# xswang/xflow

Measured on AMD Instinct MI355X. Metric: examples/sec, higher is better.
Workload: dtype f32

## Files before the change

include/xflow_amd.h:

```cpp
#ifndef XFLOW_AMD_H_
#define XFLOW_AMD_H_

#include <stddef.h>
#include <stdint.h>

#ifdef __cplusplus
extern "C" {
#endif

#define XF_OK 0
#define XF_EINVAL 1
#define XF_EHIP 2
#define XF_EFULL 3
#define XF_EIO 4
#define XF_EPARSE 5
#define XF_ENOGPU 6

const char *xf_last_error(void);
int xf_version(void);
int xf_device_count(int *count);

uint64_t xf_hash_bytes(const void *ptr, size_t len);
int xf_hash_decimal_range(uint64_t start, size_t n, uint64_t *out);
int xf_hash_decimal_ids(const uint64_t *ids, size_t n, uint64_t *out);
// ... 359 lines not shown
                   const int32_t *fgid, const float *vals, const int32_t *labels,
                   size_t row_begin, size_t row_end, void *stream, const uint64_t **d_keys_out,
                   const int32_t **d_fgid_out, const float **d_vals_out,
                   const uint32_t **d_rowptr_out, const int32_t **d_labels_out, uint32_t *R_out,
                   uint32_t *NNZ_out);
int xf_admit_export(xf_admit *a, uint8_t *counters);
int xf_admit_import(xf_admit *a, const uint8_t *counters);
int xf_admit_save(xf_admit *a, const char *path);
int xf_admit_load(xf_admit *a, const char *path);
int xf_admit_stats(const xf_admit *a, uint64_t *nonzeros_seen, uint64_t *nonzeros_kept);

typedef struct xf_negsample xf_negsample;
int xf_negsample_create(xf_negsample **out, float keep, uint64_t seed);
int xf_negsample_destroy(xf_negsample *s);
int xf_negsample_params(const xf_negsample *s, float *keep, uint64_t *seed);
int xf_negsample_weight(const xf_negsample *s, float *weight);
int xf_negsample_keep(uint64_t seed, uint64_t stream, uint64_t ordinal, float keep);
int xf_negsample_apply_dev(xf_negsample *s, uint64_t stream_id, uint64_t first_ordinal,
                           const uint64_t *d_keys, const int32_t *d_fgid, const float *d_vals,
                           const uint32_t *d_rowptr, const int32_t *d_labels, uint32_t R,
                           uint32_t NNZ, void *stream, const uint64_t **d_keys_out,
                           const int32_t **d_fgid_out, const float **d_vals_out,
                           const uint32_t **d_rowptr_out, const int32_t **d_labels_out,
                           uint32_t *R_out, uint32_t *NNZ_out);
int xf_negsample_apply(xf_negsample *s, uint64_t stream_id, uint64_t first_ordinal,
                       const uint64_t *rowptr, const uint64_t *keys, const int32_t *fgid,
                       const float *vals, const int32_t *labels, size_t row_begin, size_t row_end,
                       void *stream, const uint64_t **d_keys_out, const int32_t **d_fgid_out,
                       const float **d_vals_out, const uint32_t **d_rowptr_out,
                       const int32_t **d_labels_out, uint32_t *R_out, uint32_t *NNZ_out);
int xf_negsample_stats(const xf_negsample *s, uint64_t *rows_seen, uint64_t *rows_kept,
                       uint64_t *neg_seen, uint64_t *neg_kept);
int xf_workspace_neg_weight(xf_workspace *ws, float weight);
int xf_sharded_set_neg_weight(xf_sharded *st, float weight);

int xf_auc_logloss(const int32_t *labels, const float *pctr, size_t n,
                   float *acc_logloss_inout, float *auc, int *tp, int *fp,
                   double *nat_logloss);

int XFCreate(void **h, const char *train_path, const char *test_path);
int XFStartTrain(void **h);
int XFDestroy(void **h);
int XFSetParam(void *h, const char *name, const char *value);
int XFGetMetric(void *h, const char *name, double *value);
int XFSaveModel(void *h, const char *path);
int XFLoadModel(void *h, const char *path);
int XFPredict(void *h);
int XFGetTables(void *h, xf_table **w, xf_table **v);

#ifdef __cplusplus
}
#endif
#endif
```

xflow_amd/capi.py:

```python
import collections
import ctypes as C
import os

import numpy as np

_HERE = os.path.dirname(os.path.abspath(__file__))
LIB_PATH = os.environ.get("XF_LIB") or os.path.join(_HERE, "lib", "libxflow_amd.so")

XF_OK = 0
OPT_FTRL, OPT_SGD = 0, 1
INIT_ZERO, INIT_CONST, INIT_HASHNORM = 0, 1, 2
(DEFRAG_NONE, DEFRAG_SORTFREE, DEFRAG_RADIX_ASKED, DEFRAG_RADIX_EXTENT, DEFRAG_RADIX_COUNT,
 DEFRAG_RADIX_CLUSTER) = range(6)
HEAVY_SEG = 64
FM_REFERENCE, FM_CANONICAL, FM_FIELD_AWARE = 0, 1, 2
FM_MODES = {"reference": FM_REFERENCE, "canonical": FM_CANONICAL, "field_aware": FM_FIELD_AWARE}

u64p = C.POINTER(C.c_uint64)
u32p = C.POINTER(C.c_uint32)
i32p = C.POINTER(C.c_int32)
f32p = C.POINTER(C.c_float)
vp = C.c_void_p


# ... 223 lines not shown
    "xf_admit_range": (C.c_int, [C.c_int, C.c_int, C.c_int, u64p, u64p]),
    "xf_admit_range_of": (C.c_int, [vp, u64p, u64p]),
    "xf_admit_destroy": (C.c_int, [vp]),
    "xf_admit_params": (C.c_int, [vp, C.POINTER(C.c_int), C.POINTER(C.c_int), C.POINTER(C.c_int),
                                  C.POINTER(C.c_uint64)]),
    "xf_admit_apply_dev": (C.c_int, [vp, C.c_int, vp, vp, vp, vp, C.c_uint32, C.c_uint32, vp,
                                     C.POINTER(vp), C.POINTER(vp), C.POINTER(vp), C.POINTER(vp),
                                     C.POINTER(C.c_uint32)]),
    "xf_admit_apply": (C.c_int, [vp, C.c_int, u64p, u64p, i32p, f32p, i32p, C.c_size_t,
                                 C.c_size_t, vp, C.POINTER(vp), C.POINTER(vp), C.POINTER(vp),
                                 C.POINTER(vp), C.POINTER(vp), C.POINTER(C.c_uint32),
                                 C.POINTER(C.c_uint32)]),
    "xf_admit_export": (C.c_int, [vp, C.POINTER(C.c_uint8)]),
    "xf_admit_import": (C.c_int, [vp, C.POINTER(C.c_uint8)]),
    "xf_admit_save": (C.c_int, [vp, C.c_char_p]),
    "xf_admit_load": (C.c_int, [vp, C.c_char_p]),
    "xf_admit_stats": (C.c_int, [vp, u64p, u64p]),
    "xf_negsample_create": (C.c_int, [C.POINTER(vp), C.c_float, C.c_uint64]),
    "xf_negsample_destroy": (C.c_int, [vp]),
    "xf_negsample_params": (C.c_int, [vp, C.POINTER(C.c_float), u64p]),
    "xf_negsample_weight": (C.c_int, [vp, C.POINTER(C.c_float)]),
    "xf_negsample_keep": (C.c_int, [C.c_uint64, C.c_uint64, C.c_uint64, C.c_float]),
    "xf_negsample_apply_dev": (C.c_int, [vp, C.c_uint64, C.c_uint64, vp, vp, vp, vp, vp,
                                         C.c_uint32, C.c_uint32, vp, C.POINTER(vp),
                                         C.POINTER(vp), C.POINTER(vp), C.POINTER(vp),
                                         C.POINTER(vp), C.POINTER(C.c_uint32),
                                         C.POINTER(C.c_uint32)]),
    "xf_negsample_apply": (C.c_int, [vp, C.c_uint64, C.c_uint64, u64p, u64p, i32p, f32p, i32p,
                                     C.c_size_t, C.c_size_t, vp, C.POINTER(vp), C.POINTER(vp),
                                     C.POINTER(vp), C.POINTER(vp), C.POINTER(vp),
                                     C.POINTER(C.c_uint32), C.POINTER(C.c_uint32)]),
    "xf_negsample_stats": (C.c_int, [vp, u64p, u64p, u64p, u64p]),
    "xf_workspace_neg_weight": (C.c_int, [vp, C.c_float]),
    "xf_sharded_set_neg_weight": (C.c_int, [vp, C.c_float]),
    "XFCreate": (C.c_int, [C.POINTER(vp), C.c_char_p, C.c_char_p]),
    "XFStartTrain": (C.c_int, [C.POINTER(vp)]),
    "XFDestroy": (C.c_int, [C.POINTER(vp)]),
    "XFSetParam": (C.c_int, [vp, C.c_char_p, C.c_char_p]),
    "XFGetMetric": (C.c_int, [vp, C.c_char_p, C.POINTER(C.c_double)]),
    "XFGetTables": (C.c_int, [vp, C.POINTER(vp), C.POINTER(vp)]),
    "XFSaveModel": (C.c_int, [vp, C.c_char_p]),
    "XFLoadModel": (C.c_int, [vp, C.c_char_p]),
    "XFPredict": (C.c_int, [vp]),
}

_lib = None


def _share_hip_runtime_with_torch():
    import importlib.util
    import sys
    if "torch" in sys.modules:
        return
    try:
        spec = importlib.util.find_spec("torch")
    except (ImportError, ValueError):
        spec = None
    if spec is None or not spec.origin:
        return
    rt = os.path.join(os.path.dirname(spec.origin), "lib", "libamdhip64.so")
    if os.path.exists(rt):
        try:
            C.CDLL(rt, mode=C.RTLD_GLOBAL)
        except OSError:
            pass

# ... 1108 lines not shown
```

xflow_amd/csrc/xf_batch.cc:

```cpp
#include "xf_batch.h"
#include "xf_scratch.h"
#include "xf_tiling.h"

#include <atomic>
#include <string.h>

#include <algorithm>
#include <cmath>
#include <mutex>
#include <thread>
#include <vector>

namespace {

struct KeyPos {
  uint64_t key;
  uint32_t pos;
};

inline bool keypos_less(const KeyPos &a, const KeyPos &b) {
  return a.key < b.key || (a.key == b.key && a.pos < b.pos);
}

void sort_keypos(std::vector<KeyPos> &a) {
// ... 150 lines not shown
  if (!p) return;
  int dev = 0;
  void *evict = nullptr;
  if (hipGetDevice(&dev) == hipSuccess) {
    std::lock_guard<std::mutex> lk(g_pool_mu);
    if (g_pool_limit > 0) {
      if ((int)g_pool.size() >= g_pool_limit) {
        evict = g_pool.front().p;
        g_pool.erase(g_pool.begin());
      }
      g_pool.push_back({p, bytes, dev, false});
      p = nullptr;
    }
  }
  if (evict) (void)hipFree(evict);
  if (p) (void)hipFree(p);
}

void blob_pool_limit(int blobs) {
  std::vector<Blob> drop;
  {
    std::lock_guard<std::mutex> lk(g_pool_mu);
    g_pool_limit = blobs < 0 ? 0 : blobs;
    while ((int)g_pool.size() > g_pool_limit) {
      drop.push_back(g_pool.back());
      g_pool.pop_back();
    }
  }
  for (const Blob &b : drop) (void)hipFree(b.p);
}
}

namespace xf {
static int g_path[kPathCount] = {0, 0, 0, 0, 0};
int path_switch(int which) { return g_path[which]; }
void set_path_switch(int which, int v) { g_path[which] = v; }
#ifdef XF_EXPERIMENTS
static int g_exp_knob = 0;
int exp_knob() { return g_exp_knob; }
void set_exp_knob(int v) { g_exp_knob = v; }
#endif
static std::atomic<bool> g_device_poisoned{false};
bool device_poisoned() { return g_device_poisoned.load(std::memory_order_relaxed); }
void scratch_poison() { g_device_poisoned.store(true); }
}

extern "C" int xf_batch_pool_reserve(size_t bytes) {
  XF_REQUIRE(bytes > 0, "xf_batch_pool_reserve: no bytes");
  int dev = 0;
  XF_HIP(hipGetDevice(&dev));
  {
    std::lock_guard<std::mutex> lk(xf::g_pool_mu);
    if (xf::g_pool_limit <= 0) return XF_OK;
    for (const xf::Blob &b : xf::g_pool)
      if (b.reserved && b.dev == dev && b.bytes >= bytes) return XF_OK;
  }
  void *p = nullptr;
  XF_HIP(hipMalloc(&p, bytes));
  std::lock_guard<std::mutex> lk(xf::g_pool_mu);
  xf::g_pool.push_back({p, bytes, dev, true});
  return XF_OK;
}

extern "C" int xf_scratch_reserve(size_t bytes) {
  xf::Arena &a = xf::arena();
  XF_REQUIRE(a.used == 0, "xf_scratch_reserve: a build is in progress on this thread");
  if (bytes <= a.cap) return XF_OK;
  if (a.base) XF_HIP(hipFree(a.base));
  a.base = nullptr;
  a.cap = 0;
  XF_HIP(hipMalloc((void **)&a.base, bytes));
  a.cap = bytes;
  return XF_OK;
}

extern "C" int xf_tune(const char *name, double value) {
  XF_REQUIRE(name, "xf_tune: null name");
  if (!strcmp(name, "panel_slice_bytes")) g_panel_slice_bytes = value;
  else if (!strcmp(name, "min_panel_nnz")) g_min_panel_nnz = value;
  else if (!strcmp(name, "parse_threads")) xf::set_parse_threads((int)value);
  else if (!strcmp(name, "key_build") && value >= 0 && value <= 3)
    xf::set_path_switch(xf::kPathKeyBuild, (int)value);
  else if (!strcmp(name, "old_weight") && value >= 0 && value <= 2)
    xf::set_path_switch(xf::kPathOldWeight, (int)value);
  else if (!strcmp(name, "lr_gradient") && value >= 0 && value <= 3)
    xf::set_path_switch(xf::kPathLrGradient, (int)value);
  else if (!strcmp(name, "owner_pass") && value >= 0 && value <= 4)
    xf::set_path_switch(xf::kPathOwnerPass, (int)value);
  else if (!strcmp(name, "valued_lr") && (value == 0 || value == 1 || value == 2))
    xf::set_path_switch(xf::kPathValuedLr, (int)value);
#ifdef XF_EXPERIMENTS
  else if (!strcmp(name, "exp_knob")) xf::set_exp_knob((int)value);
#endif
  else if (!strcmp(name, "batch_pool_blobs")) xf::blob_pool_limit((int)value);
  else
    return xf::set_error(XF_EINVAL, "xf_tune: unknown knob '%s' (or a value it does not take)", name);
  return XF_OK;
}

extern "C" int xf_batch_heavy_chunks(const xf_batch *b, uint32_t *H, const uint32_t **chunk_ptr) {
  XF_REQUIRE(b && H, "xf_batch_heavy_chunks: null argument");
  XF_TRY(need_host(b));
  *H = b->H;
  if (chunk_ptr) *chunk_ptr = b->hchunk_ptr.data();
  return XF_OK;
}

extern "C" int xf_batch_tiles(const xf_batch *b, uint32_t *ntiles, const uint32_t **tile_ptr) {
  XF_REQUIRE(b && ntiles, "xf_batch_tiles: null argument");
  XF_TRY(need_host(b));
  *ntiles = (uint32_t)(b->tile_ptr.size() - 1);
  if (tile_ptr) *tile_ptr = b->tile_ptr.data();
  return XF_OK;
}

extern "C" int xf_batch_fwd_tiles(const xf_batch *b, uint32_t *ntiles, const uint32_t **tile_ptr,
                                  const uint32_t **panel_first, uint32_t *grid) {
  XF_REQUIRE(b && ntiles, "xf_batch_fwd_tiles: null argument");
  XF_TRY(need_host(b));
// ... 307 lines not shown
```

xflow_amd/csrc/xf_cells.h:

```cpp
#ifndef XF_CELLS_H_
#define XF_CELLS_H_

#include <stdint.h>

#include "xf_common.h"

namespace xf {

#ifndef XF_CHUNK_BITS
#define XF_CHUNK_BITS 11
#endif
#ifndef XF_WIN_MAX
#define XF_WIN_MAX 17408
#endif
constexpr int kChunkBits = XF_CHUNK_BITS;
constexpr uint32_t kChunk = 1u << kChunkBits;
constexpr uint32_t kWinMax = XF_WIN_MAX;
constexpr uint32_t kRowMask = 0x7FFFu;
constexpr int kTagShift = kChunkBits + 15 > 27 ? kChunkBits + 15 : 27;
constexpr uint32_t kTagMask = (1u << (32 - kTagShift)) - 1u;
static_assert(kChunkBits >= 8 && kChunkBits <= 13, "chunk of 256 .. 8192 index positions");
constexpr uint32_t kBlk = 1024;
#ifndef XF_SLICE_MAX
#define XF_SLICE_MAX (4 * kChunk > 8192 ? 4 * kChunk : 8192)
// ... 31 lines not shown
  uint8_t *item_done = nullptr;
  double *gsum = nullptr;
  uint8_t *gtouched = nullptr;
  size_t split_bytes = 0;
  mutable bool split_dirty = true;
};

namespace xf {

int cells_build(xf_cells **out, const uint32_t *d_src, const uint32_t *d_map,
                const uint32_t *d_rowptr, uint32_t R, uint32_t NNZ, uint32_t M, int mode,
                bool key_sorted_copy, hipStream_t stream, const uint32_t *d_rowid = nullptr,
                uint32_t w_fixed = 0, uint32_t chunk0 = 0, const float *d_xval = nullptr);
void cells_free(xf_cells *c);

struct KbDeferred;
int cells_build_keyed(xf_cells **out, xf_table *t, const uint64_t *d_keys,
                      const uint32_t *d_rowptr, const uint32_t *d_rowid, uint32_t R,
                      uint32_t NNZ, bool key_sorted_copy, uint32_t w_fixed, hipStream_t stream,
                      KbDeferred **defer = nullptr);
int cells_build_keyed_finish(KbDeferred *d, hipStream_t stream, bool *more);

int cells_alloc(xf_cells **out, uint32_t R, uint32_t NNZ, uint32_t M, int mode,
                bool key_sorted_copy, uint32_t w_fixed, uint32_t chunk0, bool valued = false);
int cells_plan_items(xf_cells *c, hipStream_t stream);
int cells_fill_items(xf_cells *c, uint32_t nitems, uint32_t nsplit, hipStream_t stream);
int cells_key_sorted_copy(xf_cells *c, hipStream_t stream);
uint32_t cells_split_chunks(const xf_cells *c);

size_t cells_partial_doubles(const xf_cells *c);

int cells_lr_forward(const xf_cells *c, const float *d_w, const int32_t *d_labels,
                     double *d_partial, float *d_loss, float *d_pctr, hipStream_t stream,
                     const xf_cells *resume_from = nullptr);

int cells_sort_valued(const uint32_t *cid, uint32_t *cid_s, const uint32_t *ent,
                      const float *xval, uint32_t n, int bits, uint32_t *entries, float *vals,
                      hipStream_t stream);
int cells_lr_forward_valued(const xf_cells *c, const float *d_w, const int32_t *d_labels,
                            double *d_partial, float *d_loss, float *d_pctr, hipStream_t stream);
int cells_lr_grad_update_valued(const xf_cells *c, const xf_table *t, const float *d_loss,
                                hipStream_t stream);

int cells_lr_forward_sums(const xf_cells *c, const float *d_w, double *d_partial,
                          const uint32_t *d_out_base, const uint32_t *d_out_rows,
                          double *d_rowsum, hipStream_t stream);
int cells_lr_grad_update_sources(const xf_cells *c, const xf_table *t, const float *d_loss,
                                 uint32_t n, const uint32_t *d_win, const uint32_t *d_rows,
                                 const uint32_t *d_loss_base, double *d_gsum,
                                 uint8_t *d_gtouched, hipStream_t stream,
                                 uint32_t rows_if_one = 0 );

}

#endif
```

xflow_amd/csrc/xf_cells_fwd.h:

```cpp
#ifndef XF_CELLS_FWD_H_
#define XF_CELLS_FWD_H_

#include "xf_cells_impl.h"

namespace {
__device__ __forceinline__ uint32_t cell_of(const uint32_t *__restrict__ cellptr, uint32_t lo,
                                            uint32_t hi, uint32_t j) {
  while (lo < hi) {
    const uint32_t mid = lo + (hi - lo + 1) / 2;
    if (cellptr[mid] <= j) lo = mid;
    else
      hi = mid - 1;
  }
  return lo;
}

constexpr int kFwdE = (int)(kBlk / 64);

struct FwdBlock {
  uint32_t ent[kFwdE];
  uint32_t lo, hi;
};

__device__ __forceinline__ void fwd_load(FwdBlock &B, const uint32_t *__restrict__ entries,
                                         const uint32_t *__restrict__ blk_cell, uint32_t b,
                                         uint32_t pb, uint32_t pe, uint32_t lane) {
  B.lo = blk_cell[b];
  B.hi = blk_cell[b + 1];
#pragma unroll
  for (int q = 0; q < kFwdE; ++q) {
    const uint32_t j = b * kBlk + q * 64 + lane;
    B.ent[q] = (j >= pb && j < pe) ? entries[j] : 0xFFFFFFFFu;
  }
}

}

namespace xf {
int cells_lr_finalize(const xf_cells *c, const double *d_partial, const int32_t *d_labels,
                      float *d_loss, float *d_pctr, hipStream_t s);
}

#endif
```

xflow_amd/csrc/xf_cells_fwd.hip:

```cpp
#include "xf_cells_fwd.h"

namespace {
__device__ __forceinline__ void fwd_process(const FwdBlock &B, uint32_t b, uint32_t c0,
                                            uint32_t nchunk, uint32_t lane,
                                            const uint32_t *__restrict__ cellptr,
                                            const float *__restrict__ w, double *wx) {
  const uint32_t lo = B.lo < c0 ? c0 : B.lo;
  const uint32_t hi = B.hi >= c0 + nchunk ? c0 + nchunk - 1 : B.hi;
  const bool near = hi - lo <= kTagMask;
  float wv[kFwdE];
#pragma unroll
  for (int q = 0; q < kFwdE; ++q) {
    const uint32_t e = B.ent[q];
    if (e == 0xFFFFFFFFu) continue;
    const uint32_t cell = near ? lo + (((e >> kTagShift) - (lo - c0)) & kTagMask)
                               : cell_of(cellptr, lo, hi, b * kBlk + q * 64 + lane);
    wv[q] = w[(size_t)(cell - c0) * kChunk + (e & (kChunk - 1))];
  }
#pragma unroll
  for (int q = 0; q < kFwdE; ++q) {
    const uint32_t e = B.ent[q];
    if (e != 0xFFFFFFFFu) atomicAdd(&wx[(e >> kChunkBits) & kRowMask], (double)wv[q]);
  }
}
// ... 10 lines not shown
  double *out = partial + ((size_t)v * G + g) * W;
  for (uint32_t r = tid; r < W; r += kFwdBlock) wx[r] = accumulate ? out[r] : 0.0;
  const uint32_t c0 = v * nchunk;
  const uint32_t wb = cellptr[c0], we = cellptr[c0 + nchunk];
  const uint64_t n = we - wb;
  uint32_t pb = g == 0 ? wb : (uint32_t)((wb + n * g / G) & ~(uint64_t)(kBlk - 1));
  uint32_t pe = g == G - 1 ? we : (uint32_t)((wb + n * (g + 1) / G) & ~(uint64_t)(kBlk - 1));
  if (pb < wb) pb = wb;
  if (pe < pb) pe = pb;
  const uint32_t b_first = pb / kBlk, b_end = pb < pe ? (pe - 1) / kBlk + 1 : b_first;
  if (tid == 0) next_blk = b_first;
  __syncthreads();
  auto grab = [&]() -> uint32_t {
    uint32_t b = 0;
    if (lane == 0) b = atomicAdd(&next_blk, 1u);
    return (uint32_t)__shfl((int)b, 0);
  };
  FwdBlock A, B;
  uint32_t ba = grab(), bb = 0;
  if (ba < b_end) fwd_load(A, entries, blk_cell, ba, pb, pe, lane);
  while (ba < b_end) {
    bb = grab();
    if (bb < b_end) fwd_load(B, entries, blk_cell, bb, pb, pe, lane);
    fwd_process(A, ba, c0, nchunk, lane, cellptr, w, wx);
    if (bb >= b_end) break;
    ba = grab();
    if (ba < b_end) fwd_load(A, entries, blk_cell, ba, pb, pe, lane);
    fwd_process(B, bb, c0, nchunk, lane, cellptr, w, wx);
  }
  __syncthreads();
  for (uint32_t r = tid; r < W; r += kFwdBlock) out[r] = wx[r];
}

__global__ void __launch_bounds__(kBlock)
k_lr_finalize_cells(const double *__restrict__ partial, const int32_t *__restrict__ labels,
                    uint32_t R, uint32_t W, uint32_t G, float *__restrict__ loss,
                    float *__restrict__ pctr) {
  const uint32_t t = blockIdx.x * blockDim.x + threadIdx.x;
  const uint32_t r = t >> 2, q = t & 3u;
  double a = 0.0;
  if (r < R) {
    const uint32_t v = r / W, rin = r - v * W;
    const double *p = partial + (size_t)v * G * W + rin;
    double a1 = 0.0, a2 = 0.0, a3 = 0.0;
    uint32_t g = q;
    for (; g + 12 < G; g += 16) {
      a += p[(size_t)g * W];
      a1 += p[(size_t)(g + 4) * W];
      a2 += p[(size_t)(g + 8) * W];
      a3 += p[(size_t)(g + 12) * W];
    }
    for (; g < G; g += 4) a += p[(size_t)g * W];
    a += a1 + (a2 + a3);
  }
  a += __shfl_xor(a, 1);
  a += __shfl_xor(a, 2);
  if (r >= R || q != 0) return;
  const float pr = xf::sigmoid_ref((float)a);
  if (pctr) pctr[r] = pr;
  if (loss) loss[r] = pr - (float)labels[r];
}
}

namespace xf {

int cells_lr_forward(const xf_cells *c, const float *d_w, const int32_t *d_labels,
                     double *d_partial, float *d_loss, float *d_pctr, hipStream_t s,
                     const xf_cells *resume_from) {
  XF_REQUIRE(c && d_w && d_partial && (d_loss || d_pctr), "cells_lr_forward: null argument");
  if (c->R == 0) return XF_OK;
  int acc = 0;
  const xf_cells *first = c;
  if (resume_from) {
    first = resume_from;
    acc = 1;
  }
  for (const xf_cells *q = first; q; q = q->next, acc = 1)
    hipLaunchKernelGGL(k_lr_fwd_cells, dim3(q->nwin * q->G), dim3(kFwdBlock), 0, s, q->fwd_entries(),
                       q->cellptr, q->blk_cell, q->nchunk, q->W, q->G,
                       d_w + (size_t)q->chunk0 * kChunk, d_partial, acc);
  hipLaunchKernelGGL(k_lr_finalize_cells,
                     dim3((unsigned)(((size_t)c->R * 4 + kBlock - 1) / kBlock)), dim3(kBlock), 0, s,
                     d_partial, d_labels, c->R, c->W, c->G, d_loss, d_pctr);
  XF_HIP(hipGetLastError());
  return XF_OK;
}

int cells_lr_finalize(const xf_cells *c, const double *d_partial, const int32_t *d_labels,
                      float *d_loss, float *d_pctr, hipStream_t s) {
  hipLaunchKernelGGL(k_lr_finalize_cells,
                     dim3((unsigned)(((size_t)c->R * 4 + kBlock - 1) / kBlock)), dim3(kBlock), 0, s,
                     d_partial, d_labels, c->R, c->W, c->G, d_loss, d_pctr);
  XF_HIP(hipGetLastError());
  return XF_OK;
}

namespace {
__global__ void __launch_bounds__(kBlock)
k_sum_partials(const double *__restrict__ partial, uint32_t n, uint32_t W, uint32_t G,
               const uint32_t *__restrict__ out_base, const uint32_t *__restrict__ out_rows,
               double *__restrict__ rowsum) {
  const uint32_t t = blockIdx.x * blockDim.x + threadIdx.x;
  const uint32_t r = t >> 2, q = t & 3u;
  const uint32_t v = r < n ? r / W : 0u, rin = r - v * W;
  const bool live = r < n && rin < out_rows[v];
  double a = 0.0;
  if (live) {
    const double *p = partial + (size_t)v * G * W + rin;
    for (uint32_t g = q; g < G; g += 4) a += p[(size_t)g * W];
  }
  a += __shfl_xor(a, 1);
  a += __shfl_xor(a, 2);
  if (live && q == 0) rowsum[out_base[v] + rin] = a;
}
}

int cells_lr_forward_sums(const xf_cells *c, const float *d_w, double *d_partial,
                          const uint32_t *d_out_base, const uint32_t *d_out_rows,
                          double *d_rowsum, hipStream_t s) {
  XF_REQUIRE(c && d_w && d_partial && d_rowsum && d_out_base && d_out_rows,
             "cells_lr_forward_sums: null argument");
  if (c->R == 0) return XF_OK;
  int acc = 0;
  for (const xf_cells *q = c; q; q = q->next, acc = 1)
    hipLaunchKernelGGL(k_lr_fwd_cells, dim3(q->nwin * q->G), dim3(kFwdBlock), 0, s, q->fwd_entries(),
                       q->cellptr, q->blk_cell, q->nchunk, q->W, q->G,
                       d_w + (size_t)q->chunk0 * kChunk, d_partial, acc);
  const uint32_t n = c->nwin * c->W;
  hipLaunchKernelGGL(k_sum_partials, dim3((unsigned)(((size_t)n * 4 + kBlock - 1) / kBlock)),
                     dim3(kBlock), 0, s, d_partial, n, c->W, c->G, d_out_base, d_out_rows,
                     d_rowsum);
  XF_HIP(hipGetLastError());
  return XF_OK;
}

}
```

xflow_amd/csrc/xf_cells_valued.hip:

```cpp
#include <rocprim/device/device_radix_sort.hpp>

#include "xf_cells_fwd.h"
#include "xf_cells_grad.h"

namespace {
__global__ void __launch_bounds__(kBlock)
k_cell_pack_val(const uint32_t *__restrict__ ent, const float *__restrict__ xval, size_t n,
                uint64_t *__restrict__ pay) {
  XF_GRID_STRIDE(j, n)
  pay[j] = ((uint64_t)__float_as_uint(xval[j]) << 32) | ent[j];
}

__global__ void __launch_bounds__(kBlock)
k_cell_split_val(const uint64_t *__restrict__ pay, size_t n, uint32_t *__restrict__ entries,
                 float *__restrict__ vals) {
  XF_GRID_STRIDE(j, n) {
    const uint64_t p = pay[j];
    entries[j] = (uint32_t)p;
    vals[j] = __uint_as_float((uint32_t)(p >> 32));
  }
}

struct FwdBlockV {
  FwdBlock E;
// ... 243 lines not shown
#pragma unroll
    for (int i = 0; i < 8; ++i) {
      if (!t[i]) continue;
      T.w[row0 + kb + i * kBlock + tid] = sw[i];
      if (OPT == XF_OPT_FTRL) xf::store_nz(T, row0 + kb + i * kBlock + tid, sn[i], sz[i]);
    }
  }
}
}

namespace xf {

int cells_sort_valued(const uint32_t *cid, uint32_t *cid_s, const uint32_t *ent,
                      const float *xval, uint32_t n, int bits, uint32_t *entries, float *vals,
                      hipStream_t s) {
  Scratch sc;
  uint64_t *pay = nullptr, *pay_s = nullptr;
  XF_TRY(sc.get(&pay, n));
  XF_TRY(sc.get(&pay_s, n));
  hipLaunchKernelGGL(k_cell_pack_val, dim3(grid_for((size_t)n)), dim3(kBlock), 0, s, ent, xval,
                     (size_t)n, pay);
  size_t tb = 0;
  XF_HIP(rocprim::radix_sort_pairs(nullptr, tb, cid, cid_s, pay, pay_s, (size_t)n, 0, bits, s));
  void *tmp = nullptr;
  XF_TRY(sc.get((char **)&tmp, tb));
  XF_HIP(rocprim::radix_sort_pairs(tmp, tb, cid, cid_s, pay, pay_s, (size_t)n, 0, bits, s));
  hipLaunchKernelGGL(k_cell_split_val, dim3(grid_for((size_t)n)), dim3(kBlock), 0, s, pay_s,
                     (size_t)n, entries, vals);
  XF_HIP(hipGetLastError());
  return XF_OK;
}

int cells_lr_forward_valued(const xf_cells *c, const float *d_w, const int32_t *d_labels,
                            double *d_partial, float *d_loss, float *d_pctr, hipStream_t s) {
  XF_REQUIRE(c && d_w && d_partial && (d_loss || d_pctr),
             "cells_lr_forward_valued: null argument");
  XF_REQUIRE(!c->next && c->chunk0 == 0 && c->entries_k == c->entries && (c->vals || c->NNZ == 0),
             "cells_lr_forward_valued: valued cells are one segment with their values and no "
             "key-sorted copy");
  if (c->R == 0) return XF_OK;
  hipLaunchKernelGGL(k_lr_fwd_cells_valued, dim3(c->nwin * c->G), dim3(kFwdBlock), 0, s, c->entries,
                     c->vals, c->cellptr, c->blk_cell, c->nchunk, c->W, c->G, d_w, d_partial);
  XF_HIP(hipGetLastError());
  return cells_lr_finalize(c, d_partial, d_labels, d_loss, d_pctr, s);
}

int cells_lr_grad_update_valued(const xf_cells *c, const xf_table *t, const float *d_loss,
                                hipStream_t s) {
  XF_REQUIRE(c && t && d_loss, "cells_lr_grad_update_valued: null argument");
  XF_REQUIRE(c->mode == kCellsTableRows, "cells_lr_grad_update_valued: cells are not table rows");
  XF_REQUIRE(!c->next && c->chunk0 == 0 && (c->vals || c->NNZ == 0),
             "cells_lr_grad_update_valued: valued cells are one segment with their values");
  TableDev T = table_dev(t);
  XF_REQUIRE(T.dim == 1, "cells_lr_grad_update_valued: dim must be 1");
  table_note_write(const_cast<xf_table *>(t));
  if (c->nitems == 0) return XF_OK;
  if (path_switch(kPathOldWeight) == 1) T.w_of_nz = false;
  if (c->nsplit_chunks) {
    if (c->split_dirty) XF_HIP(hipMemsetAsync(c->gsum, 0, c->split_bytes, s));
    c->split_dirty = true;
  }
  const int opt = T.nz != nullptr ? XF_OPT_FTRL : XF_OPT_SGD;
  if (opt == XF_OPT_FTRL)
    hipLaunchKernelGGL(k_lr_grad_cells_valued<XF_OPT_FTRL>, dim3(c->nitems), dim3(kBlock), 0, s, T,
                       c->entries, c->vals, c->cellptr, c->nchunk, c->nwin, c->W, c->item_chunk,
                       c->item_slice, c->item_dump, d_loss, c->R, c->M, c->gsum, c->gtouched,
                       c->chunk0);
  else
    hipLaunchKernelGGL(k_lr_grad_cells_valued<XF_OPT_SGD>, dim3(c->nitems), dim3(kBlock), 0, s, T,
                       c->entries, c->vals, c->cellptr, c->nchunk, c->nwin, c->W, c->item_chunk,
                       c->item_slice, c->item_dump, d_loss, c->R, c->M, c->gsum, c->gtouched,
                       c->chunk0);
  XF_HIP(hipGetLastError());
  XF_TRY(cells_launch_split_finish(opt, c, T, s));
  c->split_dirty = false;
  return XF_OK;
}
// ... 3 lines not shown
```

xflow_amd/csrc/xf_common.h:

```cpp
#ifndef XF_COMMON_H_
#define XF_COMMON_H_

#include <hip/hip_runtime_api.h>
#include <stdarg.h>
#include <stdint.h>
#include <stdio.h>

#include "xflow_amd.h"

namespace xf {

int set_error(int code, const char *fmt, ...);
int parse_threads();
void set_parse_threads(int n);
bool device_poisoned();
void scratch_poison();
enum PathSwitch { kPathKeyBuild = 0, kPathOldWeight, kPathLrGradient, kPathOwnerPass,
                  kPathValuedLr, kPathCount };
int path_switch(int which);
void set_path_switch(int which, int v);
inline int key_build_mode() { return path_switch(kPathKeyBuild); }
#ifdef XF_EXPERIMENTS
int exp_knob();
void set_exp_knob(int v);
#endif

#define XF_HIP(expr)                                                                  \
  do {                                                                                \
    hipError_t e__ = (expr);                                                          \
    if (e__ != hipSuccess)                                                            \
      return xf::set_error(XF_EHIP, "%s:%d %s -> %s", __FILE__, __LINE__, #expr,      \
                           hipGetErrorString(e__));                                   \
  } while (0)

#define XF_REQUIRE(cond, ...)                                   \
  do {                                                          \
    if (!(cond)) return xf::set_error(XF_EINVAL, __VA_ARGS__);  \
  } while (0)

#define XF_TRY(expr)           \
  do {                         \
    int rc__ = (expr);         \
    if (rc__ != XF_OK) return rc__; \
  } while (0)

struct ShardRange {
  uint64_t lo;
  uint64_t span;
  uint32_t shard, nshards;
};

// ... 12 lines not shown
```

xflow_amd/csrc/xf_model.hip:

```cpp
#include <hip/hip_runtime.h>

#include <math.h>

#include <algorithm>

#include "xf_batch.h"
#include "xf_cells.h"
#include "xf_common.h"
#include "xf_device.h"
#include "xf_ffm.h"
#include "xf_fm_canonical.h"
#include "xf_negsample.h"
#include "xf_scratch.h"
#include "xf_wave.h"

namespace xf {
const TableDev &table_dev(const xf_table *t);
int table_dim(const xf_table *t);
uint64_t table_uid(const xf_table *t);
uint64_t table_epoch(const xf_table *t);
int table_records(xf_table *t, size_t row_bytes, uint64_t tag, void **rec, uint64_t *gen);
uint64_t table_writes(const xf_table *t);
void table_note_write(xf_table *t);
void table_records_all_set(xf_table *t, const uint64_t key[5]);
// ... 1338 lines not shown
extern "C" int xf_fm_grad_update_dev(xf_table *tw, xf_table *tv, const xf_dev_batch *b,
                                     const uint32_t *d_rows_w, const uint32_t *d_rows_v,
                                     const float *d_wu, const float *d_vu, const float *d_vsum,
                                     const float *d_loss, float *d_gw, float *d_gv, void *stream) {
  return fm_grad_update(tw, tv, b, d_rows_w, d_rows_v, const_cast<float *>(d_wu),
                        const_cast<float *>(d_vu), d_vsum, d_loss, d_gw, d_gv, true, stream);
}

enum { kEvResolve = 0, kEvGather, kEvForward, kEvGrad, kEvUpdate, kEvCount };

struct xf_workspace {
  uint32_t *slots = nullptr, *slots2 = nullptr;
  float *wu = nullptr, *g = nullptr, *vu = nullptr, *gv = nullptr;
  float *loss = nullptr, *pctr = nullptr, *vsum = nullptr;
  void *ks = nullptr;
  void *owner_rec = nullptr;
  size_t capU = 0, capUK = 0, capR = 0;
  double *partial = nullptr;
  size_t capPartial = 0;
  float *gdense = nullptr;
  size_t capGdense = 0;
  bool capture = false;
  int parity = 0;
  int fm_mode = XF_FM_REFERENCE;
  int fm_fields = 0;
  float *fmc_S = nullptr;
  size_t capS = 0;
  float *fmc_vu = nullptr;
  size_t capVu = 0;
  double *fmc_hpart = nullptr;
  size_t capHpart = 0;
  uint32_t lastU = 0, lastR = 0;
  float neg_weight = 1.0f;
  bool profiling = false;
  static constexpr int kEvSets = 8;
  struct EvSet {
    hipEvent_t ev[kEvCount + 1] = {};
    bool pending = false;
    int nseg = 0;
    int seg_slot[kEvCount] = {};
  } sets[kEvSets];
  int cur = 0;
  static constexpr long kProfileEvery = 4;
  long step_no = 0;
  bool rec = false;
  double ms_sum[kEvCount] = {};
  long steps_timed = 0;
  int nmark = 0;
};

static int ws_reserve(xf_workspace *ws, size_t U, size_t UK, size_t R, bool fm_pooled = true) {
  auto grow = [](void **p, size_t bytes) -> hipError_t {
    if (*p) {
      hipError_t e = hipFree(*p);
      if (e != hipSuccess) return e;
    }
    return hipMalloc(p, bytes);
  };
  if (!ws->slots || U > ws->capU) {
    const size_t m = std::max<size_t>(U + U / 8, 1024);
    XF_HIP(grow((void **)&ws->slots, m * 4));
    XF_HIP(grow((void **)&ws->slots2, m * 4));
    XF_HIP(grow((void **)&ws->wu, m * 4));
    XF_HIP(grow((void **)&ws->g, m * 4));
    ws->capU = m;
  }
// ... 196 lines not shown
             "xf_workspace_capture: field-aware FM (xf_workspace_fm_mode) is not stepped with "
             "capture on: its step leaves the pulled weights and the w gradients for "
             "xf_workspace_fetch as it is");
  ws->capture = enable != 0;
  return XF_OK;
}

static int lr_step(xf_table *w, xf_batch *b, xf_workspace *ws, void *stream,
                   xf::KbDeferred *deferred) {
  struct Settle {
    xf::KbDeferred *d;
    void *stream;
    ~Settle() {
      if (d) (void)xf::cells_build_keyed_finish(d, S(stream), nullptr);
    }
  } settle{deferred, stream};
  XF_TRY(xf::ensure_cells(b, w, S(stream)));
  const xf_cells *c = b->cells;
  const bool cap = ws->capture && !b->local && b->d_rows_u;
  if (settle.d && (cap || ws->parity == XF_PARITY_REFERENCE_ORDER)) {
    xf::KbDeferred *d = settle.d;
    settle.d = nullptr;
    XF_TRY(xf::cells_build_keyed_finish(d, S(stream), nullptr));
  }
  XF_TRY(ws_reserve(ws, b->U, 0, b->R));
  XF_TRY(ws_reserve_cells(ws, c, cap));
  ws->rec = ws->profiling && ws->step_no++ % xf_workspace::kProfileEvery == 0;
  if (ws->rec) XF_TRY(ws_next_set(ws));
  ws->lastU = cap ? b->U : 0;
  ws->lastR = b->R;
  const xf::TableDev &T = xf::table_dev(w);
  const int32_t *labels = b->local ? b->raw_labels : b->view.labels;
  XF_BEGIN();
  if (ws->parity == XF_PARITY_REFERENCE_ORDER)
    XF_TRY(lr_forward_reforder(w, b, ws->loss, nullptr, S(stream)));
  else
    XF_TRY(xf::cells_lr_forward(c, T.w, labels, ws->partial, ws->loss, nullptr, S(stream)));
  if (settle.d) {
    xf::KbDeferred *d = settle.d;
    settle.d = nullptr;
    bool more = false;
    XF_TRY(xf::cells_build_keyed_finish(d, S(stream), &more));
    if (more) {
      const size_t had = ws->capPartial;
      XF_TRY(ws_reserve_cells(ws, c, cap));
      XF_TRY(xf::cells_lr_forward(c, xf::table_dev(w).w, labels, ws->partial, ws->loss, nullptr,
                                  S(stream), ws->capPartial == had ? c->next : nullptr));
    }
  }
  XF_TRY(xf::weigh_negatives(ws->loss, labels, b->R, ws->neg_weight, S(stream)));
  XF_END(kEvForward);
  if (cap) XF_TRY(xf::gather_f32(T.w, b->d_rows_u, b->U, ws->wu, S(stream)));
  if (ws->parity == XF_PARITY_REFERENCE_ORDER) {
    XF_TRY(xf::batch_reference_coo(b, S(stream)));
    if (b->U) {
      hipLaunchKernelGGL(k_lr_grad_reforder, dim3(blocks_for_groups(b->U, kBlock / 64)),
                         dim3(kBlock), 0, S(stream), b->view.segptr, b->d_ref_coo, ws->loss, b->U,
                         b->R, ws->g);
      XF_HIP(hipGetLastError());
      XF_TRY(xf_table_update_dev(w, b->d_rows_u, b->U, ws->g, stream));
    }
    XF_END(kEvGrad);
    if (ws->rec) ws->sets[ws->cur].pending = true;
    return XF_OK;
  }
  XF_TRY(xf::cells_lr_grad_update(c, w, ws->loss, cap ? ws->gdense : nullptr, S(stream)));
  XF_END(kEvGrad);
  if (cap) XF_TRY(xf::gather_f32(ws->gdense, b->d_rows_u, b->U, ws->g, S(stream)));
  if (ws->rec) ws->sets[ws->cur].pending = true;
  return XF_OK;
}

static int lr_valued_step(xf_table *w, xf_batch *b, xf_workspace *ws, void *stream);
static int lr_valued_predict(xf_table *w, xf_batch *b, xf_workspace *ws, float *pctr_out);
static int lr_local_valued_step(xf_table *w, xf_batch *b, xf_workspace *ws, void *stream);
static int lr_local_valued_predict(xf_table *w, xf_batch *b, xf_workspace *ws, float *pctr_out);

extern "C" int xf_lr_step(xf_table *w, xf_batch *b, xf_workspace *ws, void *stream) {
  XF_REQUIRE(w && b && ws, "xf_lr_step: null argument");
  XF_REQUIRE(xf::table_dim(w) == 1, "xf_lr_step: the w table must have dim 1");
  if (b->valued) return lr_valued_step(w, b, ws, stream);
  if (b->local_valued) return lr_local_valued_step(w, b, ws, stream);
  return lr_step(w, b, ws, stream, nullptr);
// ... 405 lines not shown
  if (v.U && v.R) {
    xf::table_note_write(w);
    XF_TRY(xf::val_lr_grad_update(w, &v, b->d_coo_val, b->d_fm_rows[0], ws->wu, ws->loss, ws->g,
                                  ws->fmc_hpart, S(stream)));
  }
  XF_END(kEvGrad);
  if (ws->rec) ws->sets[ws->cur].pending = true;
  return XF_OK;
}

static int lr_valued_predict(xf_table *w, xf_batch *b, xf_workspace *ws, float *pctr_out) {
  XF_TRY(valued_check(ws, "xf_lr_predict"));
  XF_TRY(xf_batch_upload(b, nullptr));
  XF_TRY(ws_reserve(ws, b->U, 0, b->R, false));
  const xf_dev_batch &v = b->view;
  XF_TRY(xf_table_pull_dev(w, v.ukeys, v.U, ws->slots, ws->wu, nullptr));
  XF_TRY(xf::val_lr_forward(&v, b->d_xval, ws->wu, ws->loss, ws->pctr, nullptr));
  if (b->R) XF_HIP(hipMemcpy(pctr_out, ws->pctr, (size_t)b->R * 4, hipMemcpyDeviceToHost));
  return xf_table_check(w, nullptr);
}

static int lr_local_valued_step(xf_table *w, xf_batch *b, xf_workspace *ws, void *stream) {
  XF_TRY(valued_check(ws, "xf_lr_step"));
  XF_TRY(xf::ensure_cells(b, w, S(stream)));
  const xf_cells *c = b->cells;
  XF_TRY(ws_reserve(ws, 0, 0, b->R));
  XF_TRY(ws_reserve_cells(ws, c, false));
  ws->rec = ws->profiling && ws->step_no++ % xf_workspace::kProfileEvery == 0;
  if (ws->rec) XF_TRY(ws_next_set(ws));
  ws->lastU = 0;
  ws->lastR = b->R;
  XF_BEGIN();
  XF_TRY(xf::cells_lr_forward_valued(c, xf::table_dev(w).w, b->raw_labels, ws->partial, ws->loss,
                                     nullptr, S(stream)));
  XF_TRY(xf::weigh_negatives(ws->loss, b->raw_labels, b->R, ws->neg_weight, S(stream)));
  XF_END(kEvForward);
  XF_TRY(xf::cells_lr_grad_update_valued(c, w, ws->loss, S(stream)));
  XF_END(kEvGrad);
  if (ws->rec) ws->sets[ws->cur].pending = true;
  return XF_OK;
}

static int lr_local_valued_predict(xf_table *w, xf_batch *b, xf_workspace *ws, float *pctr_out) {
  XF_TRY(valued_check(ws, "xf_lr_predict"));
  XF_TRY(xf::ensure_cells(b, w, nullptr));
  XF_TRY(ws_reserve(ws, 0, 0, b->R));
  XF_TRY(ws_reserve_cells(ws, b->cells, false));
  XF_TRY(xf::cells_lr_forward_valued(b->cells, xf::table_dev(w).w, b->raw_labels, ws->partial,
                                     ws->loss, ws->pctr, nullptr));
  if (b->R) XF_HIP(hipMemcpy(pctr_out, ws->pctr, (size_t)b->R * 4, hipMemcpyDeviceToHost));
  return xf_table_check(w, nullptr);
}

static int no_local_valued(const xf_batch *b, const char *who) {
  XF_REQUIRE(!b->local_valued,
             "%s: a local minibatch with feature values (xf_batch_compile_local_valued*) is "
             "stepped and scored by xf_lr_step / xf_lr_predict only: FM needs a minibatch with a "
             "key list and its value arrays (xf_batch_compile_valued*)", who);
  return XF_OK;
}

extern "C" int xf_fm_step(xf_table *w, xf_table *vt, xf_batch *b, xf_workspace *ws,
                          void *stream) {
  XF_REQUIRE(w && vt && b && ws, "xf_fm_step: null argument");
  XF_REQUIRE(xf::table_dim(w) == 1, "xf_fm_step: the w table must have dim 1");
  XF_TRY(no_local_valued(b, "xf_fm_step"));
  XF_REQUIRE(!b->local, "xf_fm_step: needs a minibatch with a key list (xf_batch_compile*)");
  if (ws->fm_mode == XF_FM_FIELD_AWARE) return fm_field_aware_step(w, vt, b, ws, stream);
// ... 321 lines not shown
```

xflow_amd/csrc/xf_negsample.hip:

```cpp
#include <hip/hip_runtime.h>

#include <rocprim/device/device_scan.hpp>

#include <math.h>

#include <vector>

#include "xf_common.h"
#include "xf_negsample.h"
#include "xflow_amd.h"

namespace {

constexpr int kNsThreads = 256;
constexpr uint32_t kNsTile = 256;
static_assert(kNsTile == kNsThreads, "a row per thread");
constexpr uint32_t kNsChunk = 2048;
constexpr int kNsPerThread = kNsChunk / kNsThreads;

__device__ inline bool ns_row(const uint32_t *__restrict__ rowptr,
                              const int32_t *__restrict__ labels, uint32_t r, uint32_t NNZ,
                              uint64_t base, uint64_t first_ordinal, uint64_t T, bool *negative,
                              uint32_t *len) {
  const uint32_t a = rowptr[r], b = rowptr[r + 1];
  *len = (b >= a && b <= NNZ) ? b - a : 0u;
  *negative = labels[r] == 0;
  return !*negative || xf::negsample_keep_row(base, first_ordinal + (uint64_t)r, T);
}

__device__ inline void ns_block_sum2(uint32_t *a, uint32_t *b, uint32_t (*lds)[kNsThreads / 64]) {
#pragma unroll
  for (int off = 32; off > 0; off >>= 1) {
    *a += __shfl_xor(*a, off, 64);
    *b += __shfl_xor(*b, off, 64);
  }
  const uint32_t t = threadIdx.x;
  if ((t & 63) == 0) {
    lds[0][t >> 6] = *a;
// ... 118 lines not shown
    }
  }
}

__global__ __launch_bounds__(256) void k_weigh_negatives(float *__restrict__ loss,
                                                          const int32_t *__restrict__ labels,
                                                          uint32_t R, float w) {
#pragma clang fp contract(off)
  const uint32_t r = blockIdx.x * blockDim.x + threadIdx.x;
  if (r >= R) return;
  if (labels[r] == 0) loss[r] = w * loss[r];
}

template <typename T>
int grow(T **p, size_t *cap, size_t need) {
  if (need <= *cap && *p) return XF_OK;
  if (*p) XF_HIP(hipFree(*p));
  *p = nullptr;
  *cap = 0;
  const size_t n = need + need / 4 + 64;
  XF_HIP(hipMalloc((void **)p, n * sizeof(T)));
  *cap = n;
  return XF_OK;
}

int check_keep(const char *who, float keep) {
  XF_REQUIRE(isfinite(keep) && keep > 0.0f && keep <= 1.0f,
             "%s: neg_keep must be in (0, 1], not %g", who, (double)keep);
  return XF_OK;
}

}

int xf::weigh_negatives(float *loss, const int32_t *labels, uint32_t R, float w, hipStream_t s) {
  if (w == 1.0f || R == 0) return XF_OK;
  XF_REQUIRE(loss && labels, "weigh_negatives: null argument");
  hipLaunchKernelGGL(k_weigh_negatives, dim3((R + 255) / 256), dim3(256), 0, s, loss, labels, R, w);
  XF_HIP(hipGetLastError());
  return XF_OK;
}

struct xf_negsample {
  float keep = 1.0f;
  uint64_t seed = 0, T = 0;
  uint64_t rows_seen = 0, rows_kept = 0, neg_seen = 0, neg_kept = 0;
  uint64_t *o_keys = nullptr;
  int32_t *o_fgid = nullptr, *o_labels = nullptr;
  float *o_vals = nullptr;
  uint32_t *o_rowptr = nullptr;
  size_t cap_keys = 0, cap_fgid = 0, cap_labels = 0, cap_vals = 0, cap_rowptr = 0;
  uint32_t *src_off = nullptr;
  uint64_t *tile_cnt = nullptr, *tile_off = nullptr;
  size_t cap_src = 0, cap_tcnt = 0, cap_toff = 0;
  char *scan_tmp = nullptr;
  size_t cap_scan = 0;
  unsigned long long *d_stat = nullptr;
  uint64_t *h_back = nullptr;
  uint64_t *u_keys = nullptr;
  int32_t *u_fgid = nullptr, *u_labels = nullptr;
  float *u_vals = nullptr;
  uint32_t *u_rowptr = nullptr;
  size_t ucap_keys = 0, ucap_fgid = 0, ucap_labels = 0, ucap_vals = 0, ucap_rowptr = 0;
  std::vector<uint32_t> h_rowptr;
};

extern "C" int xf_negsample_destroy(xf_negsample *s) {
  if (!s) return XF_OK;
  if (s->d_stat && !xf::device_poisoned()) {
    (void)hipDeviceSynchronize();
    for (void *p : {(void *)s->o_keys, (void *)s->o_fgid, (void *)s->o_labels, (void *)s->o_vals,
                    (void *)s->o_rowptr, (void *)s->src_off, (void *)s->tile_cnt,
                    (void *)s->tile_off, (void *)s->scan_tmp, (void *)s->d_stat, (void *)s->u_keys,
// ... 190 lines not shown
```

Baseline: 470.8 million.

## Fuse negative weighting into LR finalize and prefetch gradient entries in extra blocks

The LR finalize kernel now applies the negative-example loss weight itself, so the separate weigh_negatives launch is no longer needed on the cells path. When a gradient pass follows on a newly seen cell set, the same launch gets extra blocks. These blocks stream the entries_k array with vectorized loads to warm the cache for the gradient kernel. A bit test that can never fire, backed by a static_assert, keeps the compiler from dropping those loads. This costs extra memory traffic and blocks in finalize. A launch counter and a standalone finalize entry point are also exported.

```diff
diff --git a/include/xflow_amd.h b/include/xflow_amd.h
--- a/include/xflow_amd.h
+++ b/include/xflow_amd.h
@@ -415,6 +415,10 @@
 int xf_negsample_stats(const xf_negsample *s, uint64_t *rows_seen, uint64_t *rows_kept,
                        uint64_t *neg_seen, uint64_t *neg_kept);
 int xf_workspace_neg_weight(xf_workspace *ws, float weight);
+uint64_t xf_weigh_negatives_launches(void);
+int xf_cells_finalize_rows(const double *d_partial, const int32_t *d_labels, uint32_t R, uint32_t W,
+                           uint32_t G, float neg_weight, float *d_loss, float *d_pctr,
+                           void *stream);
 int xf_sharded_set_neg_weight(xf_sharded *st, float weight);
 
 int xf_auc_logloss(const int32_t *labels, const float *pctr, size_t n,
diff --git a/xflow_amd/capi.py b/xflow_amd/capi.py
--- a/xflow_amd/capi.py
+++ b/xflow_amd/capi.py
@@ -279,6 +279,9 @@
                                      C.POINTER(C.c_uint32), C.POINTER(C.c_uint32)]),
     "xf_negsample_stats": (C.c_int, [vp, u64p, u64p, u64p, u64p]),
     "xf_workspace_neg_weight": (C.c_int, [vp, C.c_float]),
+    "xf_weigh_negatives_launches": (C.c_uint64, []),
+    "xf_cells_finalize_rows": (C.c_int, [vp, vp, C.c_uint32, C.c_uint32, C.c_uint32, C.c_float,
+                                         vp, vp, vp]),
     "xf_sharded_set_neg_weight": (C.c_int, [vp, C.c_float]),
     "XFCreate": (C.c_int, [C.POINTER(vp), C.c_char_p, C.c_char_p]),
     "XFStartTrain": (C.c_int, [C.POINTER(vp)]),
diff --git a/xflow_amd/csrc/xf_batch.cc b/xflow_amd/csrc/xf_batch.cc
--- a/xflow_amd/csrc/xf_batch.cc
+++ b/xflow_amd/csrc/xf_batch.cc
@@ -206,7 +206,7 @@
 }
 
 namespace xf {
-static int g_path[kPathCount] = {0, 0, 0, 0, 0};
+static int g_path[kPathCount] = {0, 0, 0, 0, 0, 0};
 int path_switch(int which) { return g_path[which]; }
 void set_path_switch(int which, int v) { g_path[which] = v; }
 #ifdef XF_EXPERIMENTS
@@ -259,6 +259,8 @@
     xf::set_path_switch(xf::kPathOldWeight, (int)value);
   else if (!strcmp(name, "lr_gradient") && value >= 0 && value <= 3)
     xf::set_path_switch(xf::kPathLrGradient, (int)value);
+  else if (!strcmp(name, "entry_streams") && (value == 0 || value == 1))
+    xf::set_path_switch(xf::kPathEntryStreams, (int)value);
   else if (!strcmp(name, "owner_pass") && value >= 0 && value <= 4)
     xf::set_path_switch(xf::kPathOwnerPass, (int)value);
   else if (!strcmp(name, "valued_lr") && (value == 0 || value == 1 || value == 2))
diff --git a/xflow_amd/csrc/xf_cells.h b/xflow_amd/csrc/xf_cells.h
--- a/xflow_amd/csrc/xf_cells.h
+++ b/xflow_amd/csrc/xf_cells.h
@@ -87,13 +87,15 @@
 
 int cells_lr_forward(const xf_cells *c, const float *d_w, const int32_t *d_labels,
                      double *d_partial, float *d_loss, float *d_pctr, hipStream_t stream,
-                     const xf_cells *resume_from = nullptr);
+                     const xf_cells *resume_from = nullptr, bool grad_follows = false,
+                     float neg_weight = 1.0f);
 
 int cells_sort_valued(const uint32_t *cid, uint32_t *cid_s, const uint32_t *ent,
                       const float *xval, uint32_t n, int bits, uint32_t *entries, float *vals,
                       hipStream_t stream);
 int cells_lr_forward_valued(const xf_cells *c, const float *d_w, const int32_t *d_labels,
-                            double *d_partial, float *d_loss, float *d_pctr, hipStream_t stream);
+                            double *d_partial, float *d_loss, float *d_pctr, hipStream_t stream,
+                            float neg_weight = 1.0f );
 int cells_lr_grad_update_valued(const xf_cells *c, const xf_table *t, const float *d_loss,
                                 hipStream_t stream);
 
diff --git a/xflow_amd/csrc/xf_cells_fwd.h b/xflow_amd/csrc/xf_cells_fwd.h
--- a/xflow_amd/csrc/xf_cells_fwd.h
+++ b/xflow_amd/csrc/xf_cells_fwd.h
@@ -38,7 +38,7 @@
 
 namespace xf {
 int cells_lr_finalize(const xf_cells *c, const double *d_partial, const int32_t *d_labels,
-                      float *d_loss, float *d_pctr, hipStream_t s);
+                      float *d_loss, float *d_pctr, hipStream_t s, float neg_weight = 1.0f);
 }
 
 #endif
diff --git a/xflow_amd/csrc/xf_cells_fwd.hip b/xflow_amd/csrc/xf_cells_fwd.hip
--- a/xflow_amd/csrc/xf_cells_fwd.hip
+++ b/xflow_amd/csrc/xf_cells_fwd.hip
@@ -66,10 +66,29 @@
   for (uint32_t r = tid; r < W; r += kFwdBlock) out[r] = wx[r];
 }
 
+constexpr uint32_t kFetchVec = 4 * kBlock;
+static_assert(kWinMax <= 0x6000u, "the fetch blocks' impossible entry");
+
 __global__ void __launch_bounds__(kBlock)
 k_lr_finalize_cells(const double *__restrict__ partial, const int32_t *__restrict__ labels,
                     uint32_t R, uint32_t W, uint32_t G, float *__restrict__ loss,
-                    float *__restrict__ pctr) {
+                    float *__restrict__ pctr, float neg_w, uint32_t nfin,
+                    const uint4 *__restrict__ fetch, uint32_t nvec) {
+  if (blockIdx.x >= nfin) {
+    const uint32_t j0 = (blockIdx.x - nfin) * kFetchVec + threadIdx.x;
+    uint4 u[kFetchVec / kBlock];
+#pragma unroll
+    for (int i = 0; i < (int)(kFetchVec / kBlock); ++i) u[i] = fetch[min(j0 + i * kBlock, nvec - 1)];
+    uint32_t bad = 0;
+#pragma unroll
+    for (int i = 0; i < (int)(kFetchVec / kBlock); ++i)
+      bad |= (u[i].x >> 24 & u[i].x >> 25 & ~(u[i].x >> 11)) |
+             (u[i].y >> 24 & u[i].y >> 25 & ~(u[i].y >> 11)) |
+             (u[i].z >> 24 & u[i].z >> 25 & ~(u[i].z >> 11)) |
+             (u[i].w >> 24 & u[i].w >> 25 & ~(u[i].w >> 11));
+    if ((bad & 1u) && loss) loss[0] = 0.0f;
+    return;
+  }
   const uint32_t t = blockIdx.x * blockDim.x + threadIdx.x;
   const uint32_t r = t >> 2, q = t & 3u;
   double a = 0.0;
@@ -92,7 +111,32 @@
   if (r >= R || q != 0) return;
   const float pr = xf::sigmoid_ref((float)a);
   if (pctr) pctr[r] = pr;
-  if (loss) loss[r] = pr - (float)labels[r];
+  if (loss) {
+    const int32_t y = labels[r];
+    const float l = pr - (float)y;
+    loss[r] = y != 0 ? l : neg_w * l;
+  }
+}
+
+int launch_finalize(const xf_cells *c, const double *d_partial, const int32_t *d_labels,
+                    float *d_loss, float *d_pctr, float neg_w, const xf_cells *fetch_c,
+                    hipStream_t s) {
+  const uint32_t nfin = (uint32_t)(((size_t)c->R * 4 + kBlock - 1) / kBlock);
+  const uint4 *fetch = nullptr;
+  uint32_t nvec = 0;
+  if (fetch_c && fetch_c->NNZ) {
+    const uintptr_t a = (uintptr_t)fetch_c->entries;
+    const uint32_t head = (uint32_t)(((16 - (a & 15)) & 15) >> 2);
+    if (fetch_c->NNZ > head) {
+      fetch = (const uint4 *)(fetch_c->entries + head);
+      nvec = (fetch_c->NNZ - head) >> 2;
+    }
+  }
+  const uint32_t nfetch = (nvec + kFetchVec - 1) / kFetchVec;
+  hipLaunchKernelGGL(k_lr_finalize_cells, dim3(nfin + nfetch), dim3(kBlock), 0, s, d_partial,
+                     d_labels, c->R, c->W, c->G, d_loss, d_pctr, neg_w, nfin, fetch, nvec);
+  XF_HIP(hipGetLastError());
+  return XF_OK;
 }
 }
 
@@ -100,7 +144,7 @@
 
 int cells_lr_forward(const xf_cells *c, const float *d_w, const int32_t *d_labels,
                      double *d_partial, float *d_loss, float *d_pctr, hipStream_t s,
-                     const xf_cells *resume_from) {
+                     const xf_cells *resume_from, bool grad_follows, float neg_weight) {
   XF_REQUIRE(c && d_w && d_partial && (d_loss || d_pctr), "cells_lr_forward: null argument");
   if (c->R == 0) return XF_OK;
   int acc = 0;
@@ -113,20 +157,14 @@
     hipLaunchKernelGGL(k_lr_fwd_cells, dim3(q->nwin * q->G), dim3(kFwdBlock), 0, s, q->fwd_entries(),
                        q->cellptr, q->blk_cell, q->nchunk, q->W, q->G,
                        d_w + (size_t)q->chunk0 * kChunk, d_partial, acc);
-  hipLaunchKernelGGL(k_lr_finalize_cells,
-                     dim3((unsigned)(((size_t)c->R * 4 + kBlock - 1) / kBlock)), dim3(kBlock), 0, s,
-                     d_partial, d_labels, c->R, c->W, c->G, d_loss, d_pctr);
-  XF_HIP(hipGetLastError());
-  return XF_OK;
+  const bool fetch = grad_follows && !resume_from && path_switch(kPathEntryStreams) == 0 &&
+                     c->entries_k_ready && c->entries_k != c->entries;
+  return launch_finalize(c, d_partial, d_labels, d_loss, d_pctr, neg_weight, fetch ? c : nullptr, s);
 }
 
 int cells_lr_finalize(const xf_cells *c, const double *d_partial, const int32_t *d_labels,
-                      float *d_loss, float *d_pctr, hipStream_t s) {
-  hipLaunchKernelGGL(k_lr_finalize_cells,
-                     dim3((unsigned)(((size_t)c->R * 4 + kBlock - 1) / kBlock)), dim3(kBlock), 0, s,
-                     d_partial, d_labels, c->R, c->W, c->G, d_loss, d_pctr);
-  XF_HIP(hipGetLastError());
-  return XF_OK;
+                      float *d_loss, float *d_pctr, hipStream_t s, float neg_weight) {
+  return launch_finalize(c, d_partial, d_labels, d_loss, d_pctr, neg_weight, nullptr, s);
 }
 
 namespace {
@@ -169,3 +207,17 @@
 }
 
 }
+
+extern "C" int xf_cells_finalize_rows(const double *d_partial, const int32_t *d_labels, uint32_t R,
+                                      uint32_t W, uint32_t G, float neg_weight, float *d_loss,
+                                      float *d_pctr, void *stream) {
+  XF_REQUIRE(d_partial && d_labels && (d_loss || d_pctr) && W && G,
+             "xf_cells_finalize_rows: null argument");
+  if (R == 0) return XF_OK;
+  xf_cells c;
+  c.R = R;
+  c.W = W;
+  c.G = G;
+  return launch_finalize(&c, d_partial, d_labels, d_loss, d_pctr, neg_weight, nullptr,
+                         (hipStream_t)stream);
+}
diff --git a/xflow_amd/csrc/xf_cells_valued.hip b/xflow_amd/csrc/xf_cells_valued.hip
--- a/xflow_amd/csrc/xf_cells_valued.hip
+++ b/xflow_amd/csrc/xf_cells_valued.hip
@@ -299,7 +299,8 @@
 }
 
 int cells_lr_forward_valued(const xf_cells *c, const float *d_w, const int32_t *d_labels,
-                            double *d_partial, float *d_loss, float *d_pctr, hipStream_t s) {
+                            double *d_partial, float *d_loss, float *d_pctr, hipStream_t s,
+                            float neg_weight) {
   XF_REQUIRE(c && d_w && d_partial && (d_loss || d_pctr),
              "cells_lr_forward_valued: null argument");
   XF_REQUIRE(!c->next && c->chunk0 == 0 && c->entries_k == c->entries && (c->vals || c->NNZ == 0),
@@ -309,7 +310,7 @@
   hipLaunchKernelGGL(k_lr_fwd_cells_valued, dim3(c->nwin * c->G), dim3(kFwdBlock), 0, s, c->entries,
                      c->vals, c->cellptr, c->blk_cell, c->nchunk, c->W, c->G, d_w, d_partial);
   XF_HIP(hipGetLastError());
-  return cells_lr_finalize(c, d_partial, d_labels, d_loss, d_pctr, s);
+  return cells_lr_finalize(c, d_partial, d_labels, d_loss, d_pctr, s, neg_weight);
 }
 
 int cells_lr_grad_update_valued(const xf_cells *c, const xf_table *t, const float *d_loss,
diff --git a/xflow_amd/csrc/xf_common.h b/xflow_amd/csrc/xf_common.h
--- a/xflow_amd/csrc/xf_common.h
+++ b/xflow_amd/csrc/xf_common.h
@@ -16,7 +16,7 @@
 bool device_poisoned();
 void scratch_poison();
 enum PathSwitch { kPathKeyBuild = 0, kPathOldWeight, kPathLrGradient, kPathOwnerPass,
-                  kPathValuedLr, kPathCount };
+                  kPathValuedLr, kPathEntryStreams, kPathCount };
 int path_switch(int which);
 void set_path_switch(int which, int v);
 inline int key_build_mode() { return path_switch(kPathKeyBuild); }
diff --git a/xflow_amd/csrc/xf_model.hip b/xflow_amd/csrc/xf_model.hip
--- a/xflow_amd/csrc/xf_model.hip
+++ b/xflow_amd/csrc/xf_model.hip
@@ -1394,6 +1394,7 @@
   size_t capHpart = 0;
   uint32_t lastU = 0, lastR = 0;
   float neg_weight = 1.0f;
+  const xf_cells *last_cells = nullptr;
   bool profiling = false;
   static constexpr int kEvSets = 8;
   struct EvSet {
@@ -1656,10 +1657,14 @@
   const xf::TableDev &T = xf::table_dev(w);
   const int32_t *labels = b->local ? b->raw_labels : b->view.labels;
   XF_BEGIN();
-  if (ws->parity == XF_PARITY_REFERENCE_ORDER)
+  if (ws->parity == XF_PARITY_REFERENCE_ORDER) {
     XF_TRY(lr_forward_reforder(w, b, ws->loss, nullptr, S(stream)));
-  else
-    XF_TRY(xf::cells_lr_forward(c, T.w, labels, ws->partial, ws->loss, nullptr, S(stream)));
+    XF_TRY(xf::weigh_negatives(ws->loss, labels, b->R, ws->neg_weight, S(stream)));
+  } else {
+    XF_TRY(xf::cells_lr_forward(c, T.w, labels, ws->partial, ws->loss, nullptr, S(stream),
+                                nullptr, ws->last_cells != c, ws->neg_weight));
+  }
+  ws->last_cells = c;
   if (settle.d) {
     xf::KbDeferred *d = settle.d;
     settle.d = nullptr;
@@ -1669,10 +1674,10 @@
       const size_t had = ws->capPartial;
       XF_TRY(ws_reserve_cells(ws, c, cap));
       XF_TRY(xf::cells_lr_forward(c, xf::table_dev(w).w, labels, ws->partial, ws->loss, nullptr,
-                                  S(stream), ws->capPartial == had ? c->next : nullptr));
-    }
-  }
-  XF_TRY(xf::weigh_negatives(ws->loss, labels, b->R, ws->neg_weight, S(stream)));
+                                  S(stream), ws->capPartial == had ? c->next : nullptr, true,
+                                  ws->neg_weight));
+    }
+  }
   XF_END(kEvForward);
   if (cap) XF_TRY(xf::gather_f32(T.w, b->d_rows_u, b->U, ws->wu, S(stream)));
   if (ws->parity == XF_PARITY_REFERENCE_ORDER) {
@@ -2144,8 +2149,7 @@
   ws->lastR = b->R;
   XF_BEGIN();
   XF_TRY(xf::cells_lr_forward_valued(c, xf::table_dev(w).w, b->raw_labels, ws->partial, ws->loss,
-                                     nullptr, S(stream)));
-  XF_TRY(xf::weigh_negatives(ws->loss, b->raw_labels, b->R, ws->neg_weight, S(stream)));
+                                     nullptr, S(stream), ws->neg_weight));
   XF_END(kEvForward);
   XF_TRY(xf::cells_lr_grad_update_valued(c, w, ws->loss, S(stream)));
   XF_END(kEvGrad);
diff --git a/xflow_amd/csrc/xf_negsample.hip b/xflow_amd/csrc/xf_negsample.hip
--- a/xflow_amd/csrc/xf_negsample.hip
+++ b/xflow_amd/csrc/xf_negsample.hip
@@ -4,6 +4,7 @@
 
 #include <math.h>
 
+#include <atomic>
 #include <vector>
 
 #include "xf_common.h"
@@ -188,12 +189,19 @@
 
 }
 
+static std::atomic<uint64_t> g_weigh_launches{0};
+
 int xf::weigh_negatives(float *loss, const int32_t *labels, uint32_t R, float w, hipStream_t s) {
   if (w == 1.0f || R == 0) return XF_OK;
   XF_REQUIRE(loss && labels, "weigh_negatives: null argument");
   hipLaunchKernelGGL(k_weigh_negatives, dim3((R + 255) / 256), dim3(256), 0, s, loss, labels, R, w);
   XF_HIP(hipGetLastError());
-  return XF_OK;
+  g_weigh_launches.fetch_add(1, std::memory_order_relaxed);
+  return XF_OK;
+}
+
+extern "C" uint64_t xf_weigh_negatives_launches(void) {
+  return g_weigh_launches.load(std::memory_order_relaxed);
 }
 
 struct xf_negsample {
```

After: 493.7 million, median of 6. +4.9%, better.
